# Kumar2421/scrfd_arcface_facerecognition

Measured on AMD Instinct MI355X. Metric: faces/sec end-to-end (det+align+embed+match), higher is better.
Workload: dtype f16; 1 GPU; BASELINE configs[1]: SCRFD-10G + ArcFace-R50, 64 synthetic 640x640 frames per GPU per step, F=1 face/frame (max_num), 1000-entry gallery, random-init weights (seed 0); frames_per_gpu=64, gallery=1000, kernel_plan=plans/mi355x.plan, rec_group=2

## Files before the change

### scrfd_arcface_facerecognition_amd/csrc/conv.h

```cpp
#pragma once
#include "common.h"

namespace fid {

enum : int { ACT_NONE = 0, ACT_RELU = 1, ACT_PRELU = 2 };
enum : int {
    CF_RES_UP2 = 1,
    CF_BORDER = 2,
    CF_OUT_F32 = 4,
    CF_ARGMAX = 8,
};

struct ConvArgs {
    const void *in;
    const void *w;
    const void *w_alt;
    const float *bias;
    const float *slope;
    const void *res;
    void *out;
    void *out2;
    float *partial;
    const void *in2;
    unsigned in2_bytes;
    int H2, W2, Cin2_p, T2, kw2, s2, nchunk2, krow;
    unsigned long long *amax;
    int amax_col0;
    int H, W, Cin_p, Ho, Wo, Cout_p, w_rows;
    int kh, kw, stride, pad;
    int M, T, nchunk, ksteps, ksplit, ksteps_per_split;
    int act, flags, nsig;
    int res_H, res_W, res_Cp;
    int tiles_m, tiles_n;
    int rev;
    int tm_fast;
    unsigned in_bytes, w_bytes;
};

struct ConvPlan {
    int bm, bn, bk, ksplit;
    int gen, ns;
    size_t partial_bytes;
};
struct ConvVariant {
    const char *name;
    int gen, ns, bm, bn;
    int alt;
    bool rev;
    int force_ns;
    int base;
    int (*launch)(fid_ctx *, const ConvArgs &, const ConvPlan &);
    long long (*wgs)(const ConvArgs &, const ConvPlan &, int num_cus);
};
const ConvVariant *conv_variant(const ConvPlan &plan);
inline const char *conv_plan_name(const ConvPlan &plan) { const ConvVariant *v = conv_variant(plan); return v ? v->name : "?"; }
inline bool conv_fuses_shortcut(const ConvPlan &plan) { const ConvVariant *v = conv_variant(plan); return v && v->base >= 0; }
ConvPlan conv_fused_plan(ConvPlan base);
ConvPlan conv_base_plan(ConvPlan fused);
bool conv_force_match(const ConvPlan &plan, int force_gen, int force_ns);

ConvPlan conv_plan(const ConvArgs &a, int num_cus, bool allow_split);
ConvPlan conv_plan_untuned(const ConvArgs &a, int num_cus, bool allow_split);
#include <vector>
std::vector<ConvPlan> conv_candidates(const ConvArgs &a, int num_cus, bool allow_split);
int conv_launch(fid_ctx *ctx, ConvArgs a, const ConvPlan &plan);
float conv_plan_cu_share(const ConvArgs &a, const ConvPlan &plan, int num_cus);
inline bool conv_walks_reverse(const ConvPlan &plan) { const ConvVariant *v = conv_variant(plan); return v && v->rev; }
int plan_alt_kind(const ConvPlan &plan);
size_t repack_bytes(int kind, int Cout_p, int Cin_p, int taps = 9);
int repack_weights(fid_ctx *ctx, int kind, const void *src, void *dst, int Cout_p, int Cin_p, int taps = 9);

bool conv_direct_applicable(const ConvArgs &a);
int conv_direct_launch(fid_ctx *ctx, const ConvArgs &a);

bool conv_chunked_applicable(const ConvArgs &a);
int conv_chunked_launch(fid_ctx *ctx, const ConvArgs &a, int cb);

bool conv_pp_applicable(const ConvArgs &a);
int conv_pp_launch(fid_ctx *ctx, const ConvArgs &a, int cb);

bool conv_pc_applicable(const ConvArgs &a);
int conv_pc_launch(fid_ctx *ctx, const ConvArgs &a, int cb, int ring);

bool conv_pc2_applicable(const ConvArgs &a);
int conv_pc2_launch(fid_ctx *ctx, const ConvArgs &a);
bool conv_pcr_applicable(const ConvArgs &a);
int conv_pcr_launch(fid_ctx *ctx, const ConvArgs &a);

bool conv_wr_applicable(const ConvArgs &a);
bool conv_wr_resident_ok(const ConvArgs &a);
int conv_wr_launch(fid_ctx *ctx, const ConvArgs &a, int nt, int cb, int resident, int ring, bool strip = false);

bool mbf_block_applicable(int H, int W, int Cin_p, int Gp, int Cout_p, int stride, bool res);
int mbf_block_launch(fid_ctx *ctx, const void *x, const void *w1, const float *b1, const float *s1, int act1, const float *dww, const float *dwb,
                     const float *dws, int dw_act, const void *w2, const float *b2, const float *s2, int act2, bool res, void *out, int B, int H, int W,
                     int Cin_p, int Gp, int Cout_p, int stride);
bool conv_ks_applicable(const ConvArgs &a);
bool conv_ks_mosaic(const ConvArgs &a);
int conv_ks_launch(fid_ctx *ctx, const ConvArgs &a, int per_wg = 1, bool strip = false);
int conv_ks_items(const ConvArgs &a, bool strip = false);
bool conv_strip_ok(const ConvArgs &a);
int conv_strip_rows(const ConvArgs &a);
bool conv_ks_strip_applicable(const ConvArgs &a);

bool conv_s2_applicable(const ConvArgs &a);
int conv_s2_launch(fid_ctx *ctx, const ConvArgs &a);

bool conv_gw_applicable(const ConvArgs &a);
int conv_gw_launch(fid_ctx *ctx, const ConvArgs &a, int bm, int bn);

int conv_bb_launch(fid_ctx *ctx, const void *in, const void *w1, const float *b1, int ncls1, int act1, const float *s1, const void *w2, const float *b2,
                   void *out, int B, int H, int W, int act2, int rev, int Cp = 64);

bool dwpw_applicable(int Gp, int Cout_p);
int dwpw_launch(fid_ctx *ctx, const void *in, const float *dw_w, const float *dw_b, const float *dw_s, int dw_act, const void *pw_w, const float *pw_b,
                const float *pw_s, int pw_act, const void *res, void *out, int B, int H, int W, int Ho, int Wo, int Gp, int Cout_p, int stride);

bool stem_block_applicable(int H, int W);
int stem_block_launch(fid_ctx *ctx, const uint8_t *img, int B, int H, int W, const float *w0, const float *b0, const float *s0, int act0, const void *w1,
                      const float *b1, int ncls1, const float *s1, int act1, void *out, void *xe);

bool lat_fpn_applicable(int Cin_p, int H, int W, int rH, int rW, bool has_res);
int lat_fpn_launch(fid_ctx *ctx, const void *in, int B, int H, int W, int Cin_p, const void *w0, const float *b0, const void *res, int rH, int rW, const void *w1,
                   const float *b1, void *out, void *lat);
bool match_scan256_applicable(int n, int Gp, int dim, int num_cus);
int match_scan256_launch(fid_ctx *ctx, const void *q, const void *g, int n, int Gp, int dim, int col0, unsigned long long *amax);

int stem_fused_launch(fid_ctx *ctx, const uint8_t *img, int B, int H, int W, const void *w0, const float *b0, const void *w1,
                      const float *b1, const void *w2, const float *b2, void *out, int C2p);

int stem_rows_launch(fid_ctx *ctx, const uint8_t *img, int B, int H, int W, const void *w0, const float *b0, const void *w1,
                     const float *b1, const void *w2, const float *b2, void *out, int C2p);

}
```

### scrfd_arcface_facerecognition_amd/csrc/stem_rows.hip

```cpp
#include "conv.h"

namespace fid {
namespace {

typedef _Float16 half8 __attribute__((ext_vector_type(8)));
typedef _Float16 half4 __attribute__((ext_vector_type(4)));
typedef _Float16 half2v __attribute__((ext_vector_type(2)));
typedef float f32x4 __attribute__((ext_vector_type(4)));
typedef unsigned int u32x4 __attribute__((ext_vector_type(4)));
typedef unsigned int u32x2 __attribute__((ext_vector_type(2)));

constexpr int PXT = 6;
constexpr int CW2 = 13, CW1 = 15, CW0 = 17;
constexpr int PW0 = 18, PW1 = 16;
constexpr int DROW = 27, RS = 108;

struct StemRArgs {
    const uint8_t *img;
    const _Float16 *w0;
    const float *b0;
    const _Float16 *w1;
    const float *b1;
    const _Float16 *w2;
    const float *b2;
    _Float16 *out;
    int H, W, H1, W1, Hp, Wp;
    int tiles_x, tiles_y, n_tiles;
    int stagger;
    int ablate;
};

__device__ __forceinline__ int swz64(int lin) { return (lin >> 1) & 3; }
__device__ __forceinline__ void raw_barrier() { asm volatile("s_barrier" ::: "memory"); }
template <int N>
__device__ __forceinline__ float row_shl(float x) {
    return __builtin_bit_cast(float, __builtin_amdgcn_update_dpp(0, __builtin_bit_cast(int, x), 0x100 + N, 0xF, 0xF, true));
}

#ifndef STEM_WPS
#define STEM_WPS 2
#endif
#ifndef STEM_RELOAD_W1
#define STEM_RELOAD_W1 0
#endif
template <int C2P, int PY>
__global__ void __launch_bounds__(256, PY == 6 ? STEM_WPS : 2) scrfd_stem_rows(const StemRArgs a) {
    constexpr int R2 = 2 * PY + 1, R1 = R2 + 2, R0 = R2 + 4, RI = 2 * R0 + 1;
    constexpr int N0 = R0 * CW0, NF0 = (N0 + 15) / 16;
    constexpr int NF2 = C2P / 16, NG2 = 4 / NF2;
    constexpr int ROWS2 = NG2 == 1 ? R2 : PY + 1;
    constexpr int PR = PY / NG2;
    constexpr int ROWS1 = (R1 + 1) / 2;
    constexpr int ROWB2 = C2P * 2, CPP = ROWB2 / 16;
    constexpr int IN_BYTES = (RI * RS * 2 + 16 + 255) / 256 * 256;
    constexpr int C0_BYTES = (R0 + 1) * PW0 * 64, C1_BYTES = (R1 + 1) * PW1 * 64 + 256, STG_BYTES = PY * PXT * ROWB2;
    constexpr int OFF_IN = 0, OFF_C0 = IN_BYTES, OFF_C1 = OFF_C0 + C0_BYTES, OFF_STG = OFF_C1 + C1_BYTES, OFF_BIAS = OFF_STG + STG_BYTES;
    constexpr int MF0 = (NF0 + 3) / 4;
    constexpr int OFF_TAB = OFF_BIAS + 512, TAB_DW = MF0;
    constexpr int ZD = RI * RS / 2;
    static_assert(PY % 2 == 0 && OFF_TAB + TAB_DW * 1024 <= 80 * 1024, "two workgroups per CU");
    static_assert(PY != 6 || STEM_WPS < 3 || OFF_TAB + TAB_DW * 1024 <= 53 * 1024, "three workgroups per CU");
    constexpr int NDW = RI * DROW, DPT = (NDW + 255) / 256;
    extern __shared__ __attribute__((aligned(16))) char smem[];

    const int tid = threadIdx.x, lane = tid & 63, wave = __builtin_amdgcn_readfirstlane(tid >> 6);
    const int frow = lane & 15, fq = lane >> 4;

    half8 w0f[2], w1f[9], w2f[9];
    const int f1 = wave & 1, g1 = wave >> 1, f2 = wave % NF2, g2 = wave / NF2;
#pragma unroll
    for (int f = 0; f < 2; f++)
#pragma unroll
        for (int j = 0; j < 8; j++) {
            const int k = fq * 8 + j, dy = k / 10, e = k - dy * 10;
            w0f[f][j] = (k < 30 && e >= 1) ? a.w0[(f * 16 + frow) * 32 + dy * 9 + e - 1] : (_Float16)0.f;
        }
#pragma unroll
    for (int t = 0; t < 9; t++) {
        w1f[t] = *(const half8 *)(a.w1 + ((f1 * 16 + frow) * 9 + t) * 32 + fq * 8);
        w2f[t] = *(const half8 *)(a.w2 + ((f2 * 16 + frow) * 9 + t) * 32 + fq * 8);
    }
    float *sB = (float *)(smem + OFF_BIAS);
    if (tid < 32) { sB[tid] = a.b0[tid]; sB[32 + tid] = a.b1[tid]; }
    if (tid < C2P) sB[64 + tid] = a.b2[tid];
    if (tid < 4) ((unsigned *)(smem + OFF_IN))[ZD + tid] = 0u;

    int rel[4];
#pragma unroll
    for (int j = 0; j < 4; j++) {
        const int d = fq * 4 + j, dy = d / 5;
        rel[j] = dy * (RS / 2) + (d - dy * 5);
    }

    const int tiles_per_img = a.tiles_x * a.tiles_y;
    auto decode = [&](int tile, int &n, int &ty, int &tx) {
        n = tile / tiles_per_img;
        const int r = tile - n * tiles_per_img;
        ty = r / a.tiles_x; tx = r - ty * a.tiles_x;
    };
    unsigned pre[DPT];
    unsigned pre_ok = 0;
    bool pre_int = false;
    const int rowbytes = a.W * 3;
    int v_rel[DPT];
#pragma unroll
    for (int i = 0; i < DPT; i++) {
        const int d = tid + 256 * i;
        const int pr = d / DROW, dc = d - pr * DROW;
        v_rel[i] = d < NDW ? pr * rowbytes + dc * 4 : 0x7FFF0000;
        asm volatile("" : "+v"(v_rel[i]));
    }
    auto prefetch = [&](int tile) {
        int n, ty, tx;
        decode(tile, n, ty, tx);
        const int iy0 = 4 * PY * ty - 7, bx0 = 72 * tx - 24;
        const auto rs_img = __builtin_amdgcn_make_buffer_rsrc((void *)(a.img + (size_t)n * a.H * rowbytes), 0, a.H * rowbytes, 0x00020000);
        const int s_off = iy0 * rowbytes + bx0;
        const bool xin_all = bx0 >= 0 && bx0 + DROW * 4 <= rowbytes;
        pre_int = xin_all && iy0 >= 0 && iy0 + RI <= a.H;
        if (xin_all) {
#pragma unroll
            for (int i = 0; i < DPT; i++) pre[i] = __builtin_amdgcn_raw_buffer_load_b32(rs_img, v_rel[i] + s_off, 0, 0);
        } else {
#pragma unroll
            for (int i = 0; i < DPT; i++) {
                int d = tid + 256 * i;
                asm volatile("" : "+v"(d));
                const int pr = d / DROW, bx = bx0 + (d - pr * DROW) * 4;
                pre[i] = __builtin_amdgcn_raw_buffer_load_b32(rs_img, (bx >= 0 && bx + 4 <= rowbytes) ? v_rel[i] + s_off : 0x7FFF0000, 0, 0);
            }
        }
        pre_ok = 0xFFFFFFFFu;
        if (!pre_int) {
            pre_ok = 0;
#pragma unroll
            for (int i = 0; i < DPT; i++) {
                int d = tid + 256 * i;
                asm volatile("" : "+v"(d));
                const int pr = d / DROW, dc = d - pr * DROW;
                const int iy = iy0 + pr, bx = bx0 + dc * 4;
                const bool in = d < NDW && (unsigned)iy < (unsigned)a.H && bx >= 0 && bx + 4 <= rowbytes;
                pre_ok |= in ? (1u << i) : 0u;
            }
        }
    };
    auto commit = [&]() {
#pragma unroll
        for (int i = 0; i < DPT; i++) {
            const int d = tid + 256 * i;
            if (d < NDW) {
                const int pr = d / DROW, dc = d - pr * DROW;
                const unsigned v = pre[i];
                half4 h;
                h[0] = (_Float16)fmaf((float)(v & 0xFF), 2.f, -255.f);
                h[1] = (_Float16)fmaf((float)((v >> 8) & 0xFF), 2.f, -255.f);
                h[2] = (_Float16)fmaf((float)((v >> 16) & 0xFF), 2.f, -255.f);
                h[3] = (_Float16)fmaf((float)(v >> 24), 2.f, -255.f);
                if (!pre_int && !((pre_ok >> i) & 1u)) h = half4{0, 0, 0, 0};
                *(half4 *)(smem + OFF_IN + (pr * RS + dc * 4) * 2) = h;
            }
        }
    };

    auto make_pb = [&](int rot, int off, int (&pb)[2][4]) {
#pragma unroll
        for (int par = 0; par < 2; par++)
#pragma unroll
            for (int c = 0; c < 4; c++) {
                pb[par][c] = frow * 64 + ((fq ^ ((((frow + par) >> 1) + c + rot) & 3)) << 4) + off;
                asm volatile("" : "+v"(pb[par][c]));
            }
    };
    constexpr int NACC = ROWS2 > ROWS1 ? ROWS2 : ROWS1;
    f32x4 acc[NACC];
#ifndef STEM_PD
#define STEM_PD 3
#endif
    auto conv_rows = [&](const int (&pb)[2][4], auto rows_tag, auto pw_tag, const half8 (&wv)[9]) {
        constexpr int ROWS = decltype(rows_tag)::value, PWV = decltype(pw_tag)::value, PH = ROWS + 2;
        constexpr int PD = STEM_PD;
#pragma unroll
        for (int dx = 0; dx < 3; dx++) {
            half8 pq[PD + 1];
            auto load_p = [&](int r, int set) {
                const int K = r * PWV + dx;
                pq[set] = *(const half8 *)(smem + (pb[K & 1][(K >> 1) & 3] + K * 64));
            };
#pragma unroll
            for (int r = 0; r < PD; r++) load_p(r, r % (PD + 1));
#pragma unroll
            for (int r = 0; r < PH; r++) {
                if (r + PD < PH) load_p(r + PD, (r + PD) % (PD + 1));
                __builtin_amdgcn_sched_barrier(0);
#pragma unroll
                for (int dy = 0; dy < 3; dy++) {
                    const int mi = r - dy;
                    if (mi < 0 || mi >= ROWS) continue;
                    acc[mi] = __builtin_amdgcn_mfma_f32_16x16x32_f16(wv[dy * 3 + dx], pq[r % (PD + 1)], acc[mi], 0, 0, 0);
                }
                __builtin_amdgcn_sched_barrier(0);
            }
        }
    };
    using std::integral_constant;

    static_assert(OFF_C0 + C0_BYTES < 65536 && IN_BYTES < 65536, "both addresses of a fragment share one dword");
    unsigned *sT = (unsigned *)(smem + OFF_TAB) + tid;
#pragma unroll
    for (int i = 0; i < MF0; i++) {
        const int qd = (wave + 4 * i) * 16 + frow, q = qd < N0 ? qd : N0 - 1;
        const int y = q / CW0, x = q - y * CW0;
        const int lin = qd < N0 ? y * PW0 + x : R0 * PW0 + frow;
        const int ga = OFF_IN + (y * RS + 3 * x + 1) * 4;
        const int sa = OFF_C0 + lin * 64 + ((((fq >> 1)) ^ swz64(lin)) << 4) + (fq & 1) * 8;
        sT[i * 256] = (unsigned)ga | ((unsigned)sa << 16);
    }
#pragma unroll
    for (int j = 0; j < 4; j++) { rel[j] *= 4; asm volatile("" : "+v"(rel[j])); }

    int tile = blockIdx.x;
    if (tile < a.n_tiles) prefetch(tile);
    if (a.stagger > 0 && (int)blockIdx.x >= (int)gridDim.x / 2) {
        for (int i = 0; i < a.stagger; i += 100) __builtin_amdgcn_s_sleep(100);
    }

    for (; tile < a.n_tiles; tile += gridDim.x) {
        int n, ty, tx;
        decode(tile, n, ty, tx);
        const int py0 = ty * PY, px0 = tx * PXT;
        const int oy0 = 2 * py0 - 3, ox0 = 2 * px0 - 3;
        const bool interior = oy0 >= 0 && ox0 >= 0 && oy0 + R0 <= a.H1 && ox0 + CW0 + 1 <= a.W1;

        if (!(a.ablate & 16)) commit();
        {
            const int next = tile + gridDim.x;
            if (next < a.n_tiles && !(a.ablate & 16)) prefetch(next);
        }
        asm volatile("s_waitcnt lgkmcnt(0)" ::: "memory");
        raw_barrier();

        if (!(a.ablate & 1)) {
            constexpr int FB = 3;
            int lt = tid;
            asm volatile("" : "+v"(lt));
            const unsigned *tp = (const unsigned *)(smem + OFF_TAB) + lt;
            unsigned g_as[MF0];
#pragma unroll
            for (int i = 0; i < MF0; i++) g_as[i] = tp[i * 256];
            const int (&relb)[4] = rel;
            f32x4 bias0[2];
#pragma unroll
            for (int f = 0; f < 2; f++) bias0[f] = *(const f32x4 *)(sB + f * 16 + fq * 4);
#pragma unroll
            for (int i0 = 0; i0 < MF0; i0 += FB) {
                u32x4 pv[FB];
#pragma unroll
                for (int i = 0; i < FB; i++) {
                    if (i0 + i >= MF0) continue;
                    const int ga = (int)(g_as[i0 + i] & 0xFFFFu);
                    pv[i][0] = *(const unsigned *)(smem + (ga + relb[0]));
                    pv[i][1] = *(const unsigned *)(smem + (ga + relb[1]));
                    pv[i][2] = *(const unsigned *)(smem + (ga + relb[2]));
                    pv[i][3] = *(const unsigned *)(smem + (fq == 3 ? OFF_IN + ZD * 4 : ga + relb[3]));
                }
                f32x4 c[FB][2];
#pragma unroll
                for (int i = 0; i < FB; i++) {
                    if (i0 + i >= MF0 || wave + 4 * (i0 + i) >= NF0) continue;
                    const half8 pf = __builtin_bit_cast(half8, pv[i]);
#pragma unroll
                    for (int f = 0; f < 2; f++) c[i][f] = __builtin_amdgcn_mfma_f32_16x16x32_f16(w0f[f], pf, bias0[f], 0, 0, 0);
                }
#pragma unroll
                for (int i = 0; i < FB; i++) {
                    if (i0 + i >= MF0 || wave + 4 * (i0 + i) >= NF0) continue;
                    bool inside = true;
                    if (!interior) {
                        int lo = lane;
                        asm volatile("" : "+v"(lo));
                        const int qd = (wave + 4 * (i0 + i)) * 16 + (lo & 15), q = qd < N0 ? qd : N0 - 1;
                        const int y = q / CW0, x = q - y * CW0;
                        inside = (unsigned)(oy0 + y) < (unsigned)a.H1 && (unsigned)(ox0 + x) < (unsigned)a.W1;
                    }
#pragma unroll
                    for (int f = 0; f < 2; f++) {
                        half4 h = __builtin_elementwise_max(__builtin_convertvector(c[i][f], half4), half4{0, 0, 0, 0});
                        if (!inside) h = half4{0, 0, 0, 0};
                        *(half4 *)(smem + ((g_as[i0 + i] >> 16) ^ (f * 32))) = h;
                    }
                }
            }
        }
        asm volatile("s_waitcnt lgkmcnt(0)" ::: "memory");
        raw_barrier();

        if (!(a.ablate & 2)) {
            const int r_lo = g1 * ROWS1;
            int pb[2][4];
            make_pb(((r_lo * PW0) >> 1) & 3, OFF_C0 + r_lo * PW0 * 64, pb);
            {
                const f32x4 bias1 = *(const f32x4 *)(sB + 32 + f1 * 16 + fq * 4);
#pragma unroll
                for (int r = 0; r < ROWS1; r++) acc[r] = bias1;
            }
            conv_rows(pb, integral_constant<int, ROWS1>{}, integral_constant<int, PW0>{}, w1f);
            int lo = lane;
            asm volatile("" : "+v"(lo));
            const int fr = lo & 15, q4 = lo >> 4;
            const bool xin = fr < CW1 && (unsigned)(ox0 + 1 + fr) < (unsigned)a.W1;
            char *cp = smem + OFF_C1 + (r_lo * PW1 + fr) * 64 + (((f1 * 2 + (q4 >> 1)) ^ swz64(fr)) << 4) + (q4 & 1) * 8;
#pragma unroll
            for (int i = 0; i < ROWS1; i++) {
                if (r_lo + i >= R1) continue;
                half4 h = __builtin_elementwise_max(__builtin_convertvector(acc[i], half4), half4{0, 0, 0, 0});
                if (!interior && !(xin && (unsigned)(oy0 + 1 + r_lo + i) < (unsigned)a.H1)) h = half4{0, 0, 0, 0};
                *(half4 *)(cp + i * (PW1 * 64)) = h;
            }
        }
        asm volatile("s_waitcnt lgkmcnt(0)" ::: "memory");
        raw_barrier();

        if (!(a.ablate & 4)) {
            const int r_lo = g2 * PY;
            int pb[2][4];
            make_pb(0, OFF_C1 + r_lo * PW1 * 64, pb);
            {
                const f32x4 bias2 = *(const f32x4 *)(sB + 64 + f2 * 16 + fq * 4);
#pragma unroll
                for (int r = 0; r < ROWS2; r++) acc[r] = bias2;
            }
            conv_rows(pb, integral_constant<int, ROWS2>{}, integral_constant<int, PW1>{}, w2f);
            int lo = lane;
            asm volatile("" : "+v"(lo));
            const int fr = lo & 15, q4 = lo >> 4;
            const bool xin = fr < CW2 && (unsigned)(ox0 + 2 + fr) < (unsigned)a.W1;
            const int gy0 = oy0 + 2 + r_lo;
            if (!interior) {
                const float ninf = -__builtin_inff();
#pragma unroll
                for (int i = 0; i < ROWS2; i++)
                    if (!(xin && (unsigned)(gy0 + i) < (unsigned)a.H1)) acc[i] = f32x4{ninf, ninf, ninf, ninf};
            }
            const bool st = (fr & 1) == 0 && fr < 2 * PXT;
            char *sp = smem + OFF_STG + ((g2 * PR) * PXT + (fr >> 1)) * ROWB2 + (f2 * 16 + q4 * 4) * 2;
#pragma unroll
            for (int p = 0; p < PR; p++) {
                f32x4 m;
#pragma unroll
                for (int e = 0; e < 4; e++) {
                    const float v = fmaxf(fmaxf(acc[2 * p][e], acc[2 * p + 1][e]), acc[2 * p + 2][e]);
                    m[e] = fmaxf(fmaxf(v, row_shl<1>(v)), row_shl<2>(v));
                }
                const half4 h = __builtin_elementwise_max(__builtin_convertvector(m, half4), half4{0, 0, 0, 0});
                if (st) *(half4 *)(sp + p * (PXT * ROWB2)) = h;
            }
        }
        asm volatile("s_waitcnt lgkmcnt(0)" ::: "memory");
        raw_barrier();

        if (!(a.ablate & 8)) {
#pragma unroll
            for (int i = 0; i < (PY * PXT * CPP + 255) / 256; i++) {
                const int s = tid + 256 * i;
                const int pix = s / CPP, c = s - pix * CPP;
                const int p = pix / PXT, q = pix - p * PXT;
                const int gy = py0 + p, gx = px0 + q;
                if (s < PY * PXT * CPP && gy < a.Hp && gx < a.Wp)
                    *(u32x4 *)((char *)a.out + (((size_t)n * a.Hp + gy) * a.Wp + gx) * ROWB2 + c * 16) = *(const u32x4 *)(smem + OFF_STG + pix * ROWB2 + c * 16);
            }
        }
        if (STEM_RELOAD_W1 && PY == 6) {
            const _Float16 *wp = a.w1;
            asm volatile("" : "+s"(wp));
#pragma unroll
            for (int t = 0; t < 9; t++) w1f[t] = *(const half8 *)(wp + ((f1 * 16 + frow) * 9 + t) * 32 + fq * 8);
        }
    }
}


template <int C2P, int PY>
__global__ void __launch_bounds__(512, 2) scrfd_stem_roles(const StemRArgs a) {
    constexpr int R2 = 2 * PY + 1, R1 = R2 + 2, R0 = R2 + 4, RI = 2 * R0 + 1;
    constexpr int N0 = R0 * CW0, NF0 = (N0 + 15) / 16;
    constexpr int NF2 = C2P / 16, NG2 = 4 / NF2;
    constexpr int ROWS2 = NG2 == 1 ? R2 : PY + 1;
    constexpr int PR = PY / NG2;
    constexpr int ROWS1 = (R1 + 1) / 2;
    constexpr int ROWB2 = C2P * 2, CPP = ROWB2 / 16;
    constexpr int IN_BYTES = (RI * RS * 2 + 16 + 255) / 256 * 256;
    constexpr int C0_BYTES = (R0 + 1) * PW0 * 64, C1_BYTES = (R1 + 1) * PW1 * 64 + 256, STG_BYTES = PY * PXT * ROWB2;
    constexpr int OFF_IN = 0, OFF_C0 = IN_BYTES, OFF_C1 = OFF_C0 + C0_BYTES, OFF_STG = OFF_C1 + 2 * C1_BYTES, OFF_BIAS = OFF_STG + STG_BYTES;
    constexpr int ZD = RI * RS / 2;
    static_assert(PY % 2 == 0 && OFF_BIAS + 512 <= 160 * 1024, "LDS budget");
    constexpr int NDW = RI * DROW, DPT = (NDW + 255) / 256;
    extern __shared__ __attribute__((aligned(16))) char smem[];

    const int tid = threadIdx.x, lane = tid & 63, wave = __builtin_amdgcn_readfirstlane(tid >> 6);
    const int role = wave >> 2, gw = wave & 3, gtid = tid & 255;
    const int frow = lane & 15, fq = lane >> 4;
    const int f1 = gw & 1, g1 = gw >> 1, f2 = gw % NF2, g2 = gw / NF2;

    half8 w0f[2], wk[9];
#pragma unroll
    for (int f = 0; f < 2; f++)
#pragma unroll
        for (int j = 0; j < 8; j++) {
            const int k = fq * 8 + j, dy = k / 10, e = k - dy * 10;
            w0f[f][j] = (role == 0 && k < 30 && e >= 1) ? a.w0[(f * 16 + frow) * 32 + dy * 9 + e - 1] : (_Float16)0.f;
        }
#pragma unroll
    for (int t = 0; t < 9; t++)
        wk[t] = role == 0 ? *(const half8 *)(a.w1 + ((f1 * 16 + frow) * 9 + t) * 32 + fq * 8) : *(const half8 *)(a.w2 + ((f2 * 16 + frow) * 9 + t) * 32 + fq * 8);
    float *sB = (float *)(smem + OFF_BIAS);
    if (tid < 32) { sB[tid] = a.b0[tid]; sB[32 + tid] = a.b1[tid]; }
    if (tid < C2P) sB[64 + tid] = a.b2[tid];
    if (tid < 4) ((unsigned *)(smem + OFF_IN))[ZD + tid] = 0u;
    int rel[4];
#pragma unroll
    for (int j = 0; j < 4; j++) {
        const int d = fq * 4 + j, dy = d / 5;
        rel[j] = dy * (RS / 2) + (d - dy * 5);
    }

    const int tiles_per_img = a.tiles_x * a.tiles_y;
    auto decode = [&](int tile, int &n, int &ty, int &tx) {
        n = tile / tiles_per_img;
        const int r = tile - n * tiles_per_img;
        ty = r / a.tiles_x; tx = r - ty * a.tiles_x;
    };
    unsigned pre[DPT];
    unsigned pre_ok = 0;
    auto prefetch = [&](int tile) {
        int n, ty, tx;
        decode(tile, n, ty, tx);
        const int iy0 = 4 * PY * ty - 7, bx0 = 72 * tx - 24, rowbytes = a.W * 3;
        const uint8_t *base = a.img + (size_t)n * a.H * rowbytes;
        pre_ok = 0;
#pragma unroll
        for (int i = 0; i < DPT; i++) {
            const int d = gtid + 256 * i;
            const int pr = d / DROW, dc = d - pr * DROW;
            const int iy = iy0 + pr, bx = bx0 + dc * 4;
            const bool in = d < NDW && (unsigned)iy < (unsigned)a.H && bx >= 0 && bx + 4 <= rowbytes;
            pre[i] = in ? *(const unsigned *)(base + (size_t)iy * rowbytes + bx) : 0u;
            pre_ok |= in ? (1u << i) : 0u;
        }
    };
    auto commit = [&]() {
#pragma unroll
        for (int i = 0; i < DPT; i++) {
            const int d = gtid + 256 * i;
            if (d < NDW) {
                const int pr = d / DROW, dc = d - pr * DROW;
                const unsigned v = pre[i];
                half4 h;
                h[0] = (_Float16)fmaf((float)(v & 0xFF), 2.f, -255.f);
                h[1] = (_Float16)fmaf((float)((v >> 8) & 0xFF), 2.f, -255.f);
                h[2] = (_Float16)fmaf((float)((v >> 16) & 0xFF), 2.f, -255.f);
                h[3] = (_Float16)fmaf((float)(v >> 24), 2.f, -255.f);
                if (!((pre_ok >> i) & 1u)) h = half4{0, 0, 0, 0};
                *(half4 *)(smem + OFF_IN + (pr * RS + dc * 4) * 2) = h;
            }
        }
    };
    auto make_pb = [&](int rot, int off, int (&pb)[2][4]) {
#pragma unroll
        for (int par = 0; par < 2; par++)
#pragma unroll
            for (int c = 0; c < 4; c++) {
                pb[par][c] = frow * 64 + ((fq ^ ((((frow + par) >> 1) + c + rot) & 3)) << 4) + off;
                asm volatile("" : "+v"(pb[par][c]));
            }
    };
    constexpr int NACC = ROWS2 > ROWS1 ? ROWS2 : ROWS1;
    f32x4 acc[NACC];
    auto conv_cols = [&](const int (&pb)[2][4], auto rows_tag, auto pw_tag, int dx0, int dx1) {
        constexpr int ROWS = decltype(rows_tag)::value, PWV = decltype(pw_tag)::value, PH = ROWS + 2;
        constexpr int PD = STEM_PD;
#pragma unroll
        for (int dx = 0; dx < 3; dx++) {
            if (dx < dx0 || dx >= dx1) continue;
            half8 pq[PD + 1];
            auto load_p = [&](int r, int set) {
                const int K = r * PWV + dx;
                pq[set] = *(const half8 *)(smem + (pb[K & 1][(K >> 1) & 3] + K * 64));
            };
#pragma unroll
            for (int r = 0; r < PD; r++) load_p(r, r % (PD + 1));
#pragma unroll
            for (int r = 0; r < PH; r++) {
                if (r + PD < PH) load_p(r + PD, (r + PD) % (PD + 1));
                __builtin_amdgcn_sched_barrier(0);
#pragma unroll
                for (int dy = 0; dy < 3; dy++) {
                    const int mi = r - dy;
                    if (mi < 0 || mi >= ROWS) continue;
                    acc[mi] = __builtin_amdgcn_mfma_f32_16x16x32_f16(wk[dy * 3 + dx], pq[r % (PD + 1)], acc[mi], 0, 0, 0);
                }
                __builtin_amdgcn_sched_barrier(0);
            }
        }
    };
    using std::integral_constant;

    const int my_tiles = (int)blockIdx.x < a.n_tiles ? (a.n_tiles - 1 - (int)blockIdx.x) / (int)gridDim.x + 1 : 0;
    auto tile_of = [&](int i) { return (int)blockIdx.x + i * (int)gridDim.x; };
    if (role == 0 && my_tiles > 0) {
        prefetch(tile_of(0));
        commit();
        if (my_tiles > 1) prefetch(tile_of(1));
    }
    asm volatile("s_waitcnt lgkmcnt(0)" ::: "memory");
    __syncthreads();

    for (int p = 0; p <= my_tiles + 1; p++) {
        if (role == 0) {
            if (p < my_tiles && !(a.ablate & 1)) {
                int n, ty, tx;
                decode(tile_of(p), n, ty, tx);
                const int oy0 = 2 * ty * PY - 3, ox0 = 2 * tx * PXT - 3;
                constexpr int MF0 = (NF0 + 3) / 4, FB = 3;
                const unsigned *ip = (const unsigned *)(smem + OFF_IN);
                int lo = lane;
                asm volatile("" : "+v"(lo));
                const int fr_ = lo & 15, q4 = lo >> 4;
                f32x4 bias0[2];
#pragma unroll
                for (int f = 0; f < 2; f++) bias0[f] = *(const f32x4 *)(sB + f * 16 + q4 * 4);
#pragma unroll
                for (int i0 = 0; i0 < MF0; i0 += FB) {
                    u32x4 pv[FB];
                    int lin[FB];
                    bool inside[FB];
#pragma unroll
                    for (int i = 0; i < FB; i++) {
                        const int fi = gw + 4 * (i0 + i);
                        const int qd = fi * 16 + fr_, q = qd < N0 ? qd : N0 - 1;
                        const int y = q / CW0, x = q - y * CW0;
                        const int bdw = y * RS + 3 * x + 1;
                        pv[i][0] = ip[bdw + rel[0]];
                        pv[i][1] = ip[bdw + rel[1]];
                        pv[i][2] = ip[bdw + rel[2]];
                        pv[i][3] = ip[q4 == 3 ? ZD : bdw + rel[3]];
                        inside[i] = qd < N0 && (unsigned)(oy0 + y) < (unsigned)a.H1 && (unsigned)(ox0 + x) < (unsigned)a.W1;
                        lin[i] = qd < N0 ? y * PW0 + x : -1;
                    }
#pragma unroll
                    for (int i = 0; i < FB; i++) {
                        if (i0 + i >= MF0 || gw + 4 * (i0 + i) >= NF0) continue;
                        const half8 pf = __builtin_bit_cast(half8, pv[i]);
#pragma unroll
                        for (int f = 0; f < 2; f++) {
                            f32x4 c = {0.f, 0.f, 0.f, 0.f};
                            c = __builtin_amdgcn_mfma_f32_16x16x32_f16(w0f[f], pf, c, 0, 0, 0);
                            half4 h = __builtin_elementwise_max(__builtin_convertvector(c + bias0[f], half4), half4{0, 0, 0, 0});
                            if (!inside[i]) h = half4{0, 0, 0, 0};
                            if (lin[i] >= 0) *(half4 *)(smem + OFF_C0 + lin[i] * 64 + (((f * 2 + (q4 >> 1)) ^ swz64(lin[i])) << 4) + (q4 & 1) * 8) = h;
                        }
                    }
                }
            }
        } else {
            if (p >= 2 && !(a.ablate & 8)) {
                int n, ty, tx;
                decode(tile_of(p - 2), n, ty, tx);
                const int py0 = ty * PY, px0 = tx * PXT;
#pragma unroll
                for (int i = 0; i < (PY * PXT * CPP + 255) / 256; i++) {
                    const int s_ = gtid + 256 * i;
                    const int pix = s_ / CPP, c = s_ - pix * CPP;
                    const int pp = pix / PXT, q = pix - pp * PXT;
                    const int gy = py0 + pp, gx = px0 + q;
                    if (s_ < PY * PXT * CPP && gy < a.Hp && gx < a.Wp)
                        *(u32x4 *)((char *)a.out + (((size_t)n * a.Hp + gy) * a.Wp + gx) * ROWB2 + c * 16) = *(const u32x4 *)(smem + OFF_STG + pix * ROWB2 + c * 16);
                }
            }
            if (p >= 1 && p <= my_tiles && !(a.ablate & 4)) {
                int pb[2][4];
                make_pb(0, OFF_C1 + ((p - 1) & 1) * C1_BYTES + g2 * PY * PW1 * 64, pb);
#pragma unroll
                for (int r = 0; r < ROWS2; r++) acc[r] = f32x4{0.f, 0.f, 0.f, 0.f};
                conv_cols(pb, integral_constant<int, ROWS2>{}, integral_constant<int, PW1>{}, 0, 2);
            }
        }
        asm volatile("s_waitcnt lgkmcnt(0)" ::: "memory");
        raw_barrier();

        if (role == 0) {
            if (p < my_tiles) {
                int n, ty, tx;
                decode(tile_of(p), n, ty, tx);
                const int oy0 = 2 * ty * PY - 3, ox0 = 2 * tx * PXT - 3;
                const bool interior = oy0 >= 0 && ox0 >= 0 && oy0 + R0 <= a.H1 && ox0 + CW0 + 1 <= a.W1;
                if (!(a.ablate & 2)) {
                    const int r_lo = g1 * ROWS1;
                    int pb[2][4];
                    make_pb(((r_lo * PW0) >> 1) & 3, OFF_C0 + r_lo * PW0 * 64, pb);
#pragma unroll
                    for (int r = 0; r < ROWS1; r++) acc[r] = f32x4{0.f, 0.f, 0.f, 0.f};
                    conv_cols(pb, integral_constant<int, ROWS1>{}, integral_constant<int, PW0>{}, 0, 3);
                    int lo = lane;
                    asm volatile("" : "+v"(lo));
                    const int fr = lo & 15, q4 = lo >> 4;
                    const f32x4 bias1 = *(const f32x4 *)(sB + 32 + f1 * 16 + q4 * 4);
                    const bool xin = fr < CW1 && (unsigned)(ox0 + 1 + fr) < (unsigned)a.W1;
                    char *cp = smem + OFF_C1 + (p & 1) * C1_BYTES + (r_lo * PW1 + fr) * 64 + (((f1 * 2 + (q4 >> 1)) ^ swz64(fr)) << 4) + (q4 & 1) * 8;
#pragma unroll
                    for (int i = 0; i < ROWS1; i++) {
                        if (r_lo + i >= R1) continue;
                        half4 h = __builtin_elementwise_max(__builtin_convertvector(acc[i] + bias1, half4), half4{0, 0, 0, 0});
                        if (!interior && !(xin && (unsigned)(oy0 + 1 + r_lo + i) < (unsigned)a.H1)) h = half4{0, 0, 0, 0};
                        *(half4 *)(cp + i * (PW1 * 64)) = h;
                    }
                }
            }
            if (p + 1 < my_tiles && !(a.ablate & 16)) {
                commit();
                if (p + 2 < my_tiles) prefetch(tile_of(p + 2));
            }
        } else {
            if (p >= 1 && p <= my_tiles && !(a.ablate & 4)) {
                int n, ty, tx;
                decode(tile_of(p - 1), n, ty, tx);
                const int oy0 = 2 * ty * PY - 3, ox0 = 2 * tx * PXT - 3;
                const bool interior = oy0 >= 0 && ox0 >= 0 && oy0 + R0 <= a.H1 && ox0 + CW0 + 1 <= a.W1;
                const int r_lo = g2 * PY;
                int pb[2][4];
                make_pb(0, OFF_C1 + ((p - 1) & 1) * C1_BYTES + r_lo * PW1 * 64, pb);
                conv_cols(pb, integral_constant<int, ROWS2>{}, integral_constant<int, PW1>{}, 2, 3);
                int lo = lane;
                asm volatile("" : "+v"(lo));
                const int fr = lo & 15, q4 = lo >> 4;
                const f32x4 bias2 = *(const f32x4 *)(sB + 64 + f2 * 16 + q4 * 4);
                const bool xin = fr < CW2 && (unsigned)(ox0 + 2 + fr) < (unsigned)a.W1;
                const int gy0 = oy0 + 2 + r_lo;
                if (!interior) {
                    const float ninf = -__builtin_inff();
#pragma unroll
                    for (int i = 0; i < ROWS2; i++)
                        if (!(xin && (unsigned)(gy0 + i) < (unsigned)a.H1)) acc[i] = f32x4{ninf, ninf, ninf, ninf};
                }
                const bool st = (fr & 1) == 0 && fr < 2 * PXT;
                char *sp = smem + OFF_STG + ((g2 * PR) * PXT + (fr >> 1)) * ROWB2 + (f2 * 16 + q4 * 4) * 2;
#pragma unroll
                for (int pp = 0; pp < PR; pp++) {
                    f32x4 m;
#pragma unroll
                    for (int e = 0; e < 4; e++) {
                        const float v = fmaxf(fmaxf(acc[2 * pp][e], acc[2 * pp + 1][e]), acc[2 * pp + 2][e]);
                        m[e] = fmaxf(fmaxf(v, row_shl<1>(v)), row_shl<2>(v));
                    }
                    const half4 h = __builtin_elementwise_max(__builtin_convertvector(m + bias2, half4), half4{0, 0, 0, 0});
                    if (st) *(half4 *)(sp + pp * (PXT * ROWB2)) = h;
                }
            }
        }
        asm volatile("s_waitcnt lgkmcnt(0)" ::: "memory");
        raw_barrier();
    }
}

template <int C2P, int PY>
int launch_roles(fid_ctx *ctx, StemRArgs &a) {
    constexpr int R2 = 2 * PY + 1, R1 = R2 + 2, R0 = R2 + 4, RI = 2 * R0 + 1;
    constexpr int lds = (RI * RS * 2 + 16 + 255) / 256 * 256 + (R0 + 1) * PW0 * 64 + 2 * ((R1 + 1) * PW1 * 64 + 256) + PY * PXT * C2P * 2 + 512;
    a.tiles_x = cdiv(a.Wp, PXT); a.tiles_y = cdiv(a.Hp, PY);
    a.n_tiles = (a.n_tiles) * a.tiles_x * a.tiles_y;
    FID_TRY(ensure_dyn_lds(ctx, (const void *)scrfd_stem_roles<C2P, PY>, lds));
    const int grid = std::min(a.n_tiles, ctx->num_cus);
    hipLaunchKernelGGL((scrfd_stem_roles<C2P, PY>), dim3(grid), dim3(512), lds, ctx->stream, a);
    FID_HIP(hipGetLastError());
    return FID_OK;
}

template <int C2P, int PY>
int launch_rows(fid_ctx *ctx, StemRArgs &a) {
    constexpr int R2 = 2 * PY + 1, R1 = R2 + 2, R0 = R2 + 4, RI = 2 * R0 + 1;
    constexpr int MF0 = ((R0 * CW0 + 15) / 16 + 3) / 4;
    constexpr int lds = (RI * RS * 2 + 16 + 255) / 256 * 256 + (R0 + 1) * PW0 * 64 + (R1 + 1) * PW1 * 64 + 256 + PY * PXT * C2P * 2 + 512 + MF0 * 1024;
    a.tiles_x = cdiv(a.Wp, PXT); a.tiles_y = cdiv(a.Hp, PY);
    a.n_tiles = (a.n_tiles) * a.tiles_x * a.tiles_y;
    FID_TRY(ensure_dyn_lds(ctx, (const void *)scrfd_stem_rows<C2P, PY>, lds));
    const int grid = std::min(a.n_tiles, ctx->num_cus * (PY == 6 ? STEM_WPS : 2));
    hipLaunchKernelGGL((scrfd_stem_rows<C2P, PY>), dim3(grid), dim3(256), lds, ctx->stream, a);
    FID_HIP(hipGetLastError());
    return FID_OK;
}

}

int stem_rows_launch(fid_ctx *ctx, const uint8_t *img, int B, int H, int W, const void *w0, const float *b0, const void *w1,
                     const float *b1, const void *w2, const float *b2, void *out, int C2p) {
    FID_REQUIRE(H % 4 == 0 && W % 4 == 0, "fused stem: frame %dx%d not a multiple of 4", W, H);
    StemRArgs a{};
    a.img = img; a.w0 = (const _Float16 *)w0; a.b0 = b0; a.w1 = (const _Float16 *)w1; a.b1 = b1;
    a.w2 = (const _Float16 *)w2; a.b2 = b2; a.out = (_Float16 *)out;
    a.H = H; a.W = W; a.H1 = H / 2; a.W1 = W / 2; a.Hp = H / 4; a.Wp = W / 4;
    a.n_tiles = B;
    if (const char *e = getenv("FID_STEM_ABLATE")) a.ablate = atoi(e);
    a.stagger = getenv("FID_STEM_STAGGER") ? atoi(getenv("FID_STEM_STAGGER")) : 0;
    const int py = getenv("FID_STEM_PY") ? atoi(getenv("FID_STEM_PY")) : 8;
    const bool roles = getenv("FID_STEM_ROLES") != nullptr;
    if (roles && C2p == 64) return launch_roles<64, 8>(ctx, a);
    if (roles && C2p == 32) return launch_roles<32, 8>(ctx, a);
    if (C2p == 64) return py == 6 ? launch_rows<64, 6>(ctx, a) : launch_rows<64, 8>(ctx, a);
    if (C2p == 32) return py == 6 ? launch_rows<32, 6>(ctx, a) : launch_rows<32, 8>(ctx, a);
    set_error("fused stem: C2p=%d unsupported", C2p);
    return FID_E_INVALID;
}

}
```

Measured before the change: 17420 faces/s.

## Add horizontally-walking fused stem kernel that reuses overlapping columns between steps

Adds a new fused stem kernel (conv0+conv1+conv2+maxpool) in which each persistent workgroup walks along a row band in steps of 8 output pixels. It shifts the overlapping intermediate columns in LDS instead of recomputing halos per tile, carries the maxpool boundary across steps in LDS, and prefetches the next step's image slice into registers while computing the current one. A cost model picks how many segments to split each band into so the grid balances across CUs. It becomes the default stem path unless the legacy env vars are set. The trade-off is serial dependence along each band and a more complex border and segment-overlap handling.

Measured after the change: 17450 faces/s, median of 2. No clear change (+0.2%).

```diff
diff --git a/scrfd_arcface_facerecognition_amd/csrc/conv.h b/scrfd_arcface_facerecognition_amd/csrc/conv.h
--- a/scrfd_arcface_facerecognition_amd/csrc/conv.h
+++ b/scrfd_arcface_facerecognition_amd/csrc/conv.h
@@ -132,4 +132,7 @@
 int stem_rows_launch(fid_ctx *ctx, const uint8_t *img, int B, int H, int W, const void *w0, const float *b0, const void *w1,
                      const float *b1, const void *w2, const float *b2, void *out, int C2p);
 
+int stem_walk_launch(fid_ctx *ctx, const uint8_t *img, int B, int H, int W, const void *w0, const float *b0, const void *w1,
+                     const float *b1, const void *w2, const float *b2, void *out, int C2p);
+
 }
diff --git a/scrfd_arcface_facerecognition_amd/csrc/stem_rows.hip b/scrfd_arcface_facerecognition_amd/csrc/stem_rows.hip
--- a/scrfd_arcface_facerecognition_amd/csrc/stem_rows.hip
+++ b/scrfd_arcface_facerecognition_amd/csrc/stem_rows.hip
@@ -693,6 +693,9 @@
 int stem_rows_launch(fid_ctx *ctx, const uint8_t *img, int B, int H, int W, const void *w0, const float *b0, const void *w1,
                      const float *b1, const void *w2, const float *b2, void *out, int C2p) {
     FID_REQUIRE(H % 4 == 0 && W % 4 == 0, "fused stem: frame %dx%d not a multiple of 4", W, H);
+    const char *rows_env = getenv("FID_STEM_ROWS");
+    if (!(rows_env && atoi(rows_env) != 0) && !getenv("FID_STEM_PY") && !getenv("FID_STEM_ROLES"))
+        return stem_walk_launch(ctx, img, B, H, W, w0, b0, w1, b1, w2, b2, out, C2p);
     StemRArgs a{};
     a.img = img; a.w0 = (const _Float16 *)w0; a.b0 = b0; a.w1 = (const _Float16 *)w1; a.b1 = b1;
     a.w2 = (const _Float16 *)w2; a.b2 = b2; a.out = (_Float16 *)out;
diff --git a/scrfd_arcface_facerecognition_amd/csrc/stem_walk.hip b/scrfd_arcface_facerecognition_amd/csrc/stem_walk.hip
--- /dev/null
+++ b/scrfd_arcface_facerecognition_amd/csrc/stem_walk.hip
@@ -0,0 +1,430 @@
+#include "conv.h"
+
+#include <climits>
+
+namespace fid {
+namespace {
+
+typedef _Float16 half8 __attribute__((ext_vector_type(8)));
+typedef _Float16 half4 __attribute__((ext_vector_type(4)));
+typedef float f32x4 __attribute__((ext_vector_type(4)));
+typedef unsigned int u32x4 __attribute__((ext_vector_type(4)));
+
+constexpr int PXS = 8;
+constexpr int PWM = 18;
+constexpr int DROW = 25;
+#ifndef STEM_WALK_RS
+#define STEM_WALK_RS 104
+#endif
+constexpr int RS = STEM_WALK_RS;
+
+struct StemWArgs {
+    const uint8_t *img;
+    const _Float16 *w0;
+    const float *b0;
+    const _Float16 *w1;
+    const float *b1;
+    const _Float16 *w2;
+    const float *b2;
+    _Float16 *out;
+    int H, W, H1, W1, Hp, Wp;
+    int bands, segs, n_items;
+    int steps, seg_steps;
+    int stagger;
+    int ablate;
+};
+
+__device__ __forceinline__ void raw_barrier() { asm volatile("s_barrier" ::: "memory"); }
+template <int N>
+__device__ __forceinline__ float row_shl(float x) {
+    return __builtin_bit_cast(float, __builtin_amdgcn_update_dpp(0, __builtin_bit_cast(int, x), 0x100 + N, 0xF, 0xF, true));
+}
+template <int N>
+__device__ __forceinline__ float row_shr(float x) {
+    return __builtin_bit_cast(float, __builtin_amdgcn_update_dpp(0, __builtin_bit_cast(int, x), 0x110 + N, 0xF, 0xF, true));
+}
+
+#ifndef STEM_PD
+#define STEM_PD 3
+#endif
+
+template <int C2P, int PY>
+__global__ void __launch_bounds__(256, 2) scrfd_stem_walk(const StemWArgs a) {
+    constexpr int R2 = 2 * PY + 1, R1 = R2 + 2, R0 = R2 + 4, RI = 2 * R0 + 1;
+    constexpr int MF0 = (R0 + 3) / 4;
+    constexpr int NF2 = C2P / 16, NG2 = 4 / NF2;
+    constexpr int ROWS2 = NG2 == 1 ? R2 : PY + 1;
+    constexpr int PR = PY / NG2;
+    constexpr int ROWS1 = (R1 + 1) / 2;
+    constexpr int ROWB2 = C2P * 2, CPP = ROWB2 / 16;
+    constexpr int IN_BYTES = (RI * RS * 2 + 16 + 255) / 256 * 256;
+    constexpr int C0_BYTES = (R0 + 1) * PWM * 64, C1_BYTES = R1 * PWM * 64, STG_BYTES = PY * PXS * ROWB2, CAR_BYTES = 4 * PR * 64;
+    constexpr int OFF_IN = 0, OFF_C0 = IN_BYTES, OFF_C1 = OFF_C0 + C0_BYTES, OFF_STG = OFF_C1 + C1_BYTES, OFF_BIAS = OFF_STG + STG_BYTES;
+    constexpr int OFF_CAR = OFF_BIAS + 512;
+    constexpr int ZD = RI * RS / 2;
+    static_assert(PY % 2 == 0 && RS % 4 == 0 && RS >= DROW * 4 && OFF_CAR + CAR_BYTES <= 80 * 1024, "two workgroups per CU");
+    constexpr int NDW = RI * DROW, DPT = (NDW + 255) / 256;
+    extern __shared__ __attribute__((aligned(16))) char smem[];
+
+    const int tid = threadIdx.x, lane = tid & 63, wave = __builtin_amdgcn_readfirstlane(tid >> 6);
+    const int frow = lane & 15, fq = lane >> 4;
+
+    half8 w0f[2], w1f[9], w2f[9];
+    const int f1 = wave & 1, g1 = wave >> 1, f2 = wave % NF2, g2 = wave / NF2;
+#pragma unroll
+    for (int f = 0; f < 2; f++)
+#pragma unroll
+        for (int j = 0; j < 8; j++) {
+            const int k = fq * 8 + j, dy = k / 10, e = k - dy * 10;
+            w0f[f][j] = (k < 30 && e >= 1) ? a.w0[(f * 16 + frow) * 32 + dy * 9 + e - 1] : (_Float16)0.f;
+        }
+#pragma unroll
+    for (int t = 0; t < 9; t++) {
+        w1f[t] = *(const half8 *)(a.w1 + ((f1 * 16 + frow) * 9 + t) * 32 + fq * 8);
+        w2f[t] = *(const half8 *)(a.w2 + ((f2 * 16 + frow) * 9 + t) * 32 + fq * 8);
+    }
+    float *sB = (float *)(smem + OFF_BIAS);
+    if (tid < 32) { sB[tid] = a.b0[tid]; sB[32 + tid] = a.b1[tid]; }
+    if (tid < C2P) sB[64 + tid] = a.b2[tid];
+    if (tid < 4) ((unsigned *)(smem + OFF_IN))[ZD + tid] = 0u;
+
+    auto decode = [&](int item, int &n, int &ty, int &k0, int &k1) {
+        const int r = item / a.segs, s = item - r * a.segs;
+        n = r / a.bands; ty = r - n * a.bands;
+        k0 = s == 0 ? 0 : a.seg_steps + (s - 1) * (a.seg_steps - 1);
+        k1 = min(a.steps, s == 0 ? a.seg_steps : k0 + a.seg_steps - 1);
+    };
+    unsigned pre[DPT];
+    unsigned pre_ok = 0;
+    bool pre_int = false;
+    const int rowbytes = a.W * 3;
+    auto prefetch = [&](int n, int ty, int k) {
+        const int iy0 = 4 * PY * ty - 7, bx0 = 96 * k - 4;
+        const auto rs_img = __builtin_amdgcn_make_buffer_rsrc((void *)(a.img + (size_t)n * a.H * rowbytes), 0, a.H * rowbytes, 0x00020000);
+        const int s_off = iy0 * rowbytes + bx0;
+        const bool xin_all = bx0 >= 0 && bx0 + DROW * 4 <= rowbytes;
+        pre_int = xin_all && iy0 >= 0 && iy0 + RI <= a.H;
+#pragma unroll
+        for (int i = 0; i < DPT; i++) {
+            int d = tid + 256 * i;
+            asm volatile("" : "+v"(d));
+            const int pr = d / DROW, dc = d - pr * DROW, bx = bx0 + dc * 4;
+            const bool ok = d < NDW && (xin_all || (bx >= 0 && bx + 4 <= rowbytes));
+            pre[i] = __builtin_amdgcn_raw_buffer_load_b32(rs_img, ok ? pr * rowbytes + dc * 4 + s_off : 0x7FFF0000, 0, 0);
+        }
+        pre_ok = 0xFFFFFFFFu;
+        if (!pre_int) {
+            pre_ok = 0;
+#pragma unroll
+            for (int i = 0; i < DPT; i++) {
+                int d = tid + 256 * i;
+                asm volatile("" : "+v"(d));
+                const int pr = d / DROW, dc = d - pr * DROW;
+                const int iy = iy0 + pr, bx = bx0 + dc * 4;
+                const bool in = d < NDW && (unsigned)iy < (unsigned)a.H && bx >= 0 && bx + 4 <= rowbytes;
+                pre_ok |= in ? (1u << i) : 0u;
+            }
+        }
+    };
+    auto commit = [&]() {
+#pragma unroll
+        for (int i = 0; i < DPT; i++) {
+            const int d = tid + 256 * i;
+            if (d < NDW) {
+                const int pr = d / DROW, dc = d - pr * DROW;
+                const unsigned v = pre[i];
+                half4 h;
+                h[0] = (_Float16)fmaf((float)(v & 0xFF), 2.f, -255.f);
+                h[1] = (_Float16)fmaf((float)((v >> 8) & 0xFF), 2.f, -255.f);
+                h[2] = (_Float16)fmaf((float)((v >> 16) & 0xFF), 2.f, -255.f);
+                h[3] = (_Float16)fmaf((float)(v >> 24), 2.f, -255.f);
+                if (!pre_int && !((pre_ok >> i) & 1u)) h = half4{0, 0, 0, 0};
+                *(half4 *)(smem + OFF_IN + (pr * RS + dc * 4) * 2) = h;
+            }
+        }
+    };
+
+    auto make_pb = [&](int rot, int off, int (&pb)[2][4]) {
+#pragma unroll
+        for (int par = 0; par < 2; par++)
+#pragma unroll
+            for (int c = 0; c < 4; c++) {
+                pb[par][c] = frow * 64 + ((fq ^ ((((frow + par) >> 1) + c + rot) & 3)) << 4) + off;
+                asm volatile("" : "+v"(pb[par][c]));
+            }
+    };
+    constexpr int NACC = ROWS2 > ROWS1 ? ROWS2 : ROWS1;
+    f32x4 acc[NACC];
+    auto conv_rows = [&](const int (&pb)[2][4], auto rows_tag, const half8 (&wv)[9]) {
+        constexpr int ROWS = decltype(rows_tag)::value, PH = ROWS + 2;
+        constexpr int PD = STEM_PD;
+#pragma unroll
+        for (int dx = 0; dx < 3; dx++) {
+            half8 pq[PD + 1];
+            auto load_p = [&](int r, int set) {
+                const int K = r * PWM + dx;
+                pq[set] = *(const half8 *)(smem + (pb[K & 1][(K >> 1) & 3] + K * 64));
+            };
+#pragma unroll
+            for (int r = 0; r < PD; r++) load_p(r, r % (PD + 1));
+#pragma unroll
+            for (int r = 0; r < PH; r++) {
+                if (r + PD < PH) load_p(r + PD, (r + PD) % (PD + 1));
+                __builtin_amdgcn_sched_barrier(0);
+#pragma unroll
+                for (int dy = 0; dy < 3; dy++) {
+                    const int mi = r - dy;
+                    if (mi < 0 || mi >= ROWS) continue;
+                    acc[mi] = __builtin_amdgcn_mfma_f32_16x16x32_f16(wv[dy * 3 + dx], pq[r % (PD + 1)], acc[mi], 0, 0, 0);
+                }
+                __builtin_amdgcn_sched_barrier(0);
+            }
+        }
+    };
+    using std::integral_constant;
+
+    const int grid = (int)gridDim.x;
+    int item = blockIdx.x, n = 0, ty = 0, k0 = 0, k1 = 0, k = 0;
+    if (item < a.n_items) {
+        decode(item, n, ty, k0, k1);
+        k = k0 > 0 ? k0 - 1 : 0;
+        if (!(a.ablate & 16)) prefetch(n, ty, k);
+    }
+    if (a.stagger > 0 && (int)blockIdx.x >= grid / 2) {
+        for (int i = 0; i < a.stagger; i += 100) __builtin_amdgcn_s_sleep(100);
+    }
+
+    bool first = true;
+    while (item < a.n_items) {
+        const bool last = k + 1 >= k1;
+        int nitem = item, nn = n, nty = ty, nk0 = k0, nk1 = k1, nk = k + 1;
+        if (last) {
+            nitem = item + grid;
+            if (nitem < a.n_items) {
+                decode(nitem, nn, nty, nk0, nk1);
+                nk = nk0 > 0 ? nk0 - 1 : 0;
+            }
+        }
+        const int py0 = ty * PY;
+        const int oy0 = 2 * py0 - 3, x0 = 16 * k;
+        const bool interior = oy0 >= 0 && oy0 + R0 <= a.H1 && k >= 1 && x0 + 16 <= a.W1;
+
+        if (!(a.ablate & 16)) {
+            commit();
+            if (nitem < a.n_items) prefetch(nn, nty, nk);
+        }
+        constexpr int NC0 = R0 * 8, NC1 = R1 * 8;
+        if (first) {
+#pragma unroll
+            for (int i = 0; i < (NC0 + NC1 + 255) / 256; i++) {
+                const int t = tid + 256 * i;
+                const bool m1 = t >= NC0;
+                const int u = m1 ? t - NC0 : t;
+                if (t < NC0 + NC1) *(u32x4 *)(smem + (m1 ? OFF_C1 : OFF_C0) + ((u >> 3) * PWM) * 64 + (u & 7) * 16) = u32x4{0, 0, 0, 0};
+            }
+        }
+        asm volatile("s_waitcnt lgkmcnt(0)" ::: "memory");
+        raw_barrier();
+
+        if (!(a.ablate & 1)) {
+            constexpr int FB = 3;
+            int lo = lane;
+            asm volatile("" : "+v"(lo));
+            const int fr = lo & 15, q4 = lo >> 4;
+            const int ga0 = OFF_IN + wave * (RS * 4) + fr * 12;
+            const int sa0 = OFF_C0 + (wave * PWM + 2 + fr) * 64 + (((q4 >> 1) ^ ((wave + 1 + (fr >> 1)) & 3)) << 4) + (q4 & 1) * 8;
+            const bool xin = x0 + fr < a.W1;
+            int rel[4];
+#pragma unroll
+            for (int j = 0; j < 4; j++) {
+                const int d = q4 * 4 + j, dy = d / 5;
+                rel[j] = (dy * (RS / 2) + (d - dy * 5)) * 4;
+            }
+            f32x4 bias0[2];
+#pragma unroll
+            for (int f = 0; f < 2; f++) bias0[f] = *(const f32x4 *)(sB + f * 16 + q4 * 4);
+#pragma unroll
+            for (int i0 = 0; i0 < MF0; i0 += FB) {
+                u32x4 pv[FB];
+#pragma unroll
+                for (int i = 0; i < FB; i++) {
+                    if (i0 + i >= MF0) continue;
+                    const int ga = wave + 4 * (i0 + i) < R0 ? ga0 + (i0 + i) * (4 * RS * 4) : ga0;
+                    pv[i][0] = *(const unsigned *)(smem + (ga + rel[0]));
+                    pv[i][1] = *(const unsigned *)(smem + (ga + rel[1]));
+                    pv[i][2] = *(const unsigned *)(smem + (ga + rel[2]));
+                    pv[i][3] = *(const unsigned *)(smem + (q4 == 3 ? OFF_IN + ZD * 4 : ga + rel[3]));
+                }
+                f32x4 c[FB][2];
+#pragma unroll
+                for (int i = 0; i < FB; i++) {
+                    if (i0 + i >= MF0 || wave + 4 * (i0 + i) >= R0) continue;
+                    const half8 pf = __builtin_bit_cast(half8, pv[i]);
+#pragma unroll
+                    for (int f = 0; f < 2; f++) c[i][f] = __builtin_amdgcn_mfma_f32_16x16x32_f16(w0f[f], pf, bias0[f], 0, 0, 0);
+                }
+#pragma unroll
+                for (int i = 0; i < FB; i++) {
+                    if (i0 + i >= MF0 || wave + 4 * (i0 + i) >= R0) continue;
+                    const bool inside = interior || (xin && (unsigned)(oy0 + wave + 4 * (i0 + i)) < (unsigned)a.H1);
+#pragma unroll
+                    for (int f = 0; f < 2; f++) {
+                        half4 h = __builtin_elementwise_max(__builtin_convertvector(c[i][f], half4), half4{0, 0, 0, 0});
+                        if (!inside) h = half4{0, 0, 0, 0};
+                        *(half4 *)(smem + ((sa0 + (i0 + i) * (4 * PWM * 64)) ^ (f * 32))) = h;
+                    }
+                }
+            }
+        }
+        asm volatile("s_waitcnt lgkmcnt(0)" ::: "memory");
+        raw_barrier();
+
+        if (!(a.ablate & 2)) {
+            const int r_lo = g1 * ROWS1;
+            int pb[2][4];
+            make_pb(((r_lo * PWM) >> 1) & 3, OFF_C0 + r_lo * PWM * 64, pb);
+            {
+                const f32x4 bias1 = *(const f32x4 *)(sB + 32 + f1 * 16 + fq * 4);
+#pragma unroll
+                for (int r = 0; r < ROWS1; r++) acc[r] = bias1;
+            }
+            conv_rows(pb, integral_constant<int, ROWS1>{}, w1f);
+            int lo = lane;
+            asm volatile("" : "+v"(lo));
+            const int fr = lo & 15, q4 = lo >> 4;
+            const bool xin = (unsigned)(x0 - 1 + fr) < (unsigned)a.W1;
+            const int grp = f1 * 2 + (q4 >> 1), hs = r_lo + 1 + (fr >> 1);
+            char *cp = smem + OFF_C1 + (r_lo * PWM + 2 + fr) * 64 + (q4 & 1) * 8;
+#pragma unroll
+            for (int i = 0; i < ROWS1; i++) {
+                if (r_lo + i >= R1) continue;
+                half4 h = __builtin_elementwise_max(__builtin_convertvector(acc[i], half4), half4{0, 0, 0, 0});
+                if (!interior && !(xin && (unsigned)(oy0 + 1 + r_lo + i) < (unsigned)a.H1)) h = half4{0, 0, 0, 0};
+                *(half4 *)(cp + i * (PWM * 64) + ((grp ^ ((hs + i) & 3)) << 4)) = h;
+            }
+        }
+        asm volatile("s_waitcnt lgkmcnt(0)" ::: "memory");
+        raw_barrier();
+
+        if (!(a.ablate & 4)) {
+            const int r_lo = g2 * PY;
+            int pb[2][4];
+            make_pb(((r_lo * PWM) >> 1) & 3, OFF_C1 + r_lo * PWM * 64, pb);
+            {
+                const f32x4 bias2 = *(const f32x4 *)(sB + 64 + f2 * 16 + fq * 4);
+#pragma unroll
+                for (int r = 0; r < ROWS2; r++) acc[r] = bias2;
+            }
+            conv_rows(pb, integral_constant<int, ROWS2>{}, w2f);
+            int lo = lane;
+            asm volatile("" : "+v"(lo));
+            const int fr = lo & 15, q4 = lo >> 4;
+            const bool xin = (unsigned)(x0 - 2 + fr) < (unsigned)a.W1;
+            const int gy0 = oy0 + 2 + r_lo;
+            const float ninf = -__builtin_inff();
+            if (!interior) {
+#pragma unroll
+                for (int i = 0; i < ROWS2; i++)
+                    if (!(xin && (unsigned)(gy0 + i) < (unsigned)a.H1)) acc[i] = f32x4{ninf, ninf, ninf, ninf};
+            }
+            f32x4 *car = (f32x4 *)(smem + OFF_CAR) + (wave * PR) * 4 + q4;
+            const bool st = (fr & 1) == 0;
+            char *sp = smem + OFF_STG + ((g2 * PR) * PXS + (fr >> 1)) * ROWB2 + (f2 * 16 + q4 * 4) * 2;
+#pragma unroll
+            for (int p = 0; p < PR; p++) {
+                f32x4 cin = f32x4{ninf, ninf, ninf, ninf};
+                if (!first) cin = car[p * 4];
+                f32x4 v, m;
+#pragma unroll
+                for (int e = 0; e < 4; e++) {
+                    v[e] = fmaxf(fmaxf(acc[2 * p][e], acc[2 * p + 1][e]), acc[2 * p + 2][e]);
+                    const float l = fr == 0 ? cin[e] : row_shr<1>(v[e]);
+                    m[e] = fmaxf(fmaxf(l, v[e]), row_shl<1>(v[e]));
+                }
+                if (fr == 15) car[p * 4] = v;
+                const half4 h = __builtin_elementwise_max(__builtin_convertvector(m, half4), half4{0, 0, 0, 0});
+                if (st) *(half4 *)(sp + p * (PXS * ROWB2)) = h;
+            }
+        }
+        asm volatile("s_waitcnt lgkmcnt(0)" ::: "memory");
+        raw_barrier();
+
+        if (k >= k0 && !(a.ablate & 8)) {
+#pragma unroll
+            for (int i = 0; i < (PY * PXS * CPP + 255) / 256; i++) {
+                const int s = tid + 256 * i;
+                const int pix = s / CPP, c = s - pix * CPP;
+                const int p = pix / PXS, q = pix - p * PXS;
+                const int gy = py0 + p, gx = PXS * k - 1 + q;
+                if (s < PY * PXS * CPP && gy < a.Hp && (unsigned)gx < (unsigned)a.Wp)
+                    *(u32x4 *)((char *)a.out + (((size_t)n * a.Hp + gy) * a.Wp + gx) * ROWB2 + c * 16) = *(const u32x4 *)(smem + OFF_STG + pix * ROWB2 + c * 16);
+            }
+        }
+        if (!last) {
+#pragma unroll
+            for (int i = 0; i < (NC0 + NC1 + 255) / 256; i++) {
+                const int t = tid + 256 * i;
+                const bool m1 = t >= NC0;
+                const int u = m1 ? t - NC0 : t;
+                if (t < NC0 + NC1) {
+                    char *src = smem + (m1 ? OFF_C1 : OFF_C0) + ((u >> 3) * PWM + 16) * 64 + (u & 7) * 16;
+                    *(u32x4 *)(src - 16 * 64) = *(const u32x4 *)src;
+                }
+            }
+        }
+        first = last;
+        item = nitem; n = nn; ty = nty; k0 = nk0; k1 = nk1; k = nk;
+    }
+}
+
+template <int C2P, int PY>
+int launch_walk(fid_ctx *ctx, StemWArgs &a, int B) {
+    constexpr int R2 = 2 * PY + 1, R1 = R2 + 2, R0 = R2 + 4, RI = 2 * R0 + 1;
+    constexpr int lds = (RI * RS * 2 + 16 + 255) / 256 * 256 + (R0 + 1) * PWM * 64 + R1 * PWM * 64 + PY * PXS * C2P * 2 + 512 + 4 * (PY / (64 / C2P)) * 64;
+    const int slots = ctx->num_cus * 2;
+    a.bands = cdiv(a.Hp, PY);
+    a.steps = a.Wp / PXS + 1;
+    auto seg_steps = [&](int S) { return cdiv(a.steps + S - 1, S); };
+    auto valid = [&](int S) {
+        const int T = seg_steps(S);
+        return S == 1 || (T >= 2 && T + (S - 2) * (T - 1) < a.steps);
+    };
+    int S = 1;
+    if (const char *e = getenv("FID_STEM_SEGS")) {
+        S = std::max(1, std::min(atoi(e), a.steps));
+        while (!valid(S)) S--;
+    } else {
+        long best = LONG_MAX;
+        for (int s = 1; s <= a.steps; s++) {
+            if (!valid(s)) continue;
+            const long cost = (long)cdiv(B * a.bands * s, slots) * seg_steps(s);
+            if (cost < best) { best = cost; S = s; }
+        }
+    }
+    a.segs = S; a.seg_steps = seg_steps(S);
+    a.n_items = B * a.bands * S;
+    FID_TRY(ensure_dyn_lds(ctx, (const void *)scrfd_stem_walk<C2P, PY>, lds));
+    const int grid = std::min(a.n_items, slots);
+    hipLaunchKernelGGL((scrfd_stem_walk<C2P, PY>), dim3(grid), dim3(256), lds, ctx->stream, a);
+    FID_HIP(hipGetLastError());
+    return FID_OK;
+}
+
+}
+
+int stem_walk_launch(fid_ctx *ctx, const uint8_t *img, int B, int H, int W, const void *w0, const float *b0, const void *w1,
+                     const float *b1, const void *w2, const float *b2, void *out, int C2p) {
+    FID_REQUIRE(H % 4 == 0 && W % 4 == 0, "fused stem: frame %dx%d not a multiple of 4", W, H);
+    StemWArgs a{};
+    a.img = img; a.w0 = (const _Float16 *)w0; a.b0 = b0; a.w1 = (const _Float16 *)w1; a.b1 = b1;
+    a.w2 = (const _Float16 *)w2; a.b2 = b2; a.out = (_Float16 *)out;
+    a.H = H; a.W = W; a.H1 = H / 2; a.W1 = W / 2; a.Hp = H / 4; a.Wp = W / 4;
+    if (const char *e = getenv("FID_STEM_ABLATE")) a.ablate = atoi(e);
+    a.stagger = getenv("FID_STEM_STAGGER") ? atoi(getenv("FID_STEM_STAGGER")) : 0;
+    if (C2p == 64) return launch_walk<64, 8>(ctx, a, B);
+    if (C2p == 32) return launch_walk<32, 8>(ctx, a, B);
+    set_error("fused stem: C2p=%d unsupported", C2p);
+    return FID_E_INVALID;
+}
+
+}
```
